# caoql98/LKGD

Hardware: AMD Instinct MI355X
Metric: denoised frames/sec (14f x 576x1024, 25-step Euler) (higher is better)
Workload: dtype f16; 1 GPU; SVD 14 frames x 576x1024, 25 Euler steps, CFG 1.0->3.0, single clip, vanilla pipeline_stable_video_diffusion_trans loop (configs[1]); unet=random-init SVD shapes (320,640,1280,1280), heads (5,10,20,20), 1.52 B params, parallelism=single GPU

## Files before the change

### lkgd_amd/csrc/gemm_wide.hip

```cpp
#include "gemm_common.h"

#ifdef WIDE_X_NOSTORE
#define WIDE_STORE_GUARD if (p.ldc < 0)
#elif defined(WIDE_X_ONELANE)
#define WIDE_STORE_GUARD if ((threadIdx.x & 63) == 0)
#else
#define WIDE_STORE_GUARD
#endif
#ifdef WIDE_X_SMALLOUT
#define WIDE_OUT_ROW(m) ((m) & 2047)
#else
#define WIDE_OUT_ROW(m) (m)
#endif
#ifdef WIDE_X_SMALLA
#define WIDE_A_ROW(m) ((m) & 4095)
#else
#define WIDE_A_ROW(m) (m)
#endif
#ifdef WIDE_X_NT
#define WIDE_ST(ptr, v) __builtin_nontemporal_store(v, ptr)
#else
#define WIDE_ST(ptr, v) (*(ptr) = (v))
#endif
#define WIDE_OUT_PITCH 336
#define WBM 256
#define WBN 320
#define WNT 512
#define WSTAGE_BYTES ((WBM + WBN) * BK * 2)
#define WBIAS_OFF (2 * WSTAGE_BYTES)
#define WRB_OFF (WBIAS_OFF + 2 * WBN * 4)
#define WRB_STRIP 768
#define WLDS (WRB_OFF + 4 * WRB_STRIP)

#define WIDE_WAIT_TOP "s_waitcnt lgkmcnt(0)\n\t"
#ifdef WIDE_X_NOSTAGE
#define WIDE_LD(X) ""
#else
#define WIDE_LD(X) X
#endif
#ifdef WIDE_X_NOREAD
#define WIDE_RD(X) ""
#else
#define WIDE_RD(X) X
#endif
#ifdef WIDE_X_NOMFMA
#define WIDE_MM(X) ""
#else
#define WIDE_MM(X) X
#endif
#if defined(WIDE_X_NOBAR) || defined(WIDE_X_STAMPS)
#define WIDE_BAR(X) ""
#else
#define WIDE_BAR(X) X
#endif
#include "gemm_wide_ktile.inc"

struct WideIn {
  unsigned oB[5];
  const half_t* wk;
};

template <bool FIRST, int NF, int MF>
__device__ __forceinline__ void wide_ktile_a(half8_t (&x1)[4], half8_t& w0, int xa0, int xa1, int wa0, int wa1,
                                             const half_t* const (&pA)[4], const WideIn& in, int m_a) {
  half8_t x0, x1_, x2, x3, w1;
#define WIDE_STMT(BODY)                                                                                                \
  asm volatile(BODY                                                                                                    \
               : "=&v"(x0), "=&v"(x1_), "=&v"(x2), "=&v"(x3), "=&v"(x1[0]), "=&v"(x1[1]), "=&v"(x1[2]), "=&v"(x1[3]),  \
                 "=&v"(w0), "=&v"(w1)                                                                                  \
               : "v"(xa0), "v"(xa1), "v"(wa0), "v"(wa1), "v"(pA[0]), "v"(pA[1]), "v"(pA[2]), "v"(pA[3]),               \
                 "v"(in.oB[0]), "v"(in.oB[1]), "v"(in.oB[2]), "v"(in.oB[3]), "v"(in.oB[4]), "s"(in.wk), "s"(m_a)       \
               : "memory", "scc", WIDE_AGPR_CLOBBERS)
  if (MF == 3) {
    if (NF == 8) {
      if (FIRST) {
        WIDE_STMT(WIDE8_M3_KTILE_ASM_FIRST_A);
      } else {
        WIDE_STMT(WIDE8_M3_KTILE_ASM_NEXT_A);
      }
    } else if (FIRST) {
      WIDE_STMT(WIDE_M3_KTILE_ASM_FIRST_A);
    } else {
      WIDE_STMT(WIDE_M3_KTILE_ASM_NEXT_A);
    }
  } else if (NF == 8) {
    if (FIRST) {
      WIDE_STMT(WIDE8_KTILE_ASM_FIRST_A);
    } else {
      WIDE_STMT(WIDE8_KTILE_ASM_NEXT_A);
    }
  } else if (FIRST) {
    WIDE_STMT(WIDE_KTILE_ASM_FIRST_A);
  } else {
    WIDE_STMT(WIDE_KTILE_ASM_NEXT_A);
  }
#undef WIDE_STMT
}

template <int NF, int MF>
__device__ __forceinline__ void wide_ktile_b(const half8_t (&x1)[4], half8_t w0, int wa1) {
  half8_t w1;
#define WIDE_STMT_B(BODY)                                                  \
  asm volatile(BODY                                                        \
               : "=&v"(w1), "+v"(w0)                                       \
               : "v"(x1[0]), "v"(x1[1]), "v"(x1[2]), "v"(x1[3]), "v"(wa1)  \
               : "memory", WIDE_AGPR_CLOBBERS)
  if (MF == 3) {
    if (NF == 8) WIDE_STMT_B(WIDE8_M3_KTILE_ASM_B);
    else WIDE_STMT_B(WIDE_M3_KTILE_ASM_B);
  } else if (NF == 8)
    asm volatile(WIDE8_KTILE_ASM_B
                 : "=&v"(w1), "+v"(w0)
                 : "v"(x1[0]), "v"(x1[1]), "v"(x1[2]), "v"(x1[3]), "v"(wa1)
                 : "memory", WIDE_AGPR_CLOBBERS);
  else
    asm volatile(WIDE_KTILE_ASM_B
                 : "=&v"(w1), "+v"(w0)
                 : "v"(x1[0]), "v"(x1[1]), "v"(x1[2]), "v"(x1[3]), "v"(wa1)
                 : "memory", WIDE_AGPR_CLOBBERS);
#undef WIDE_STMT_B
}

template <int BASE>
__device__ __forceinline__ float4_t wide_read_acc() {
  float a, b, c, d;
  asm volatile("v_accvgpr_read_b32 %0, a[%4]\n\tv_accvgpr_read_b32 %1, a[%4+1]\n\t"
               "v_accvgpr_read_b32 %2, a[%4+2]\n\tv_accvgpr_read_b32 %3, a[%4+3]"
               : "=v"(a), "=v"(b), "=v"(c), "=v"(d)
               : "i"(BASE));
  return (float4_t){a, b, c, d};
}

template <int V> struct WideIC { static constexpr int value = V; };
template <class F, int... Is> __device__ __forceinline__ void wide_static_for(F&& f, WideIC<Is>...) { (f(WideIC<Is>{}), ...); }
template <class F> __device__ __forceinline__ void wide_for10(F&& f) {
  wide_static_for(f, WideIC<0>{}, WideIC<1>{}, WideIC<2>{}, WideIC<3>{}, WideIC<4>{}, WideIC<5>{}, WideIC<6>{}, WideIC<7>{}, WideIC<8>{}, WideIC<9>{});
}
template <class F> __device__ __forceinline__ void wide_for8(F&& f) {
  wide_static_for(f, WideIC<0>{}, WideIC<1>{}, WideIC<2>{}, WideIC<3>{}, WideIC<4>{}, WideIC<5>{}, WideIC<6>{}, WideIC<7>{});
}
template <int NF, class F> __device__ __forceinline__ void wide_for_nf(F&& f) {
  if constexpr (NF == 8) wide_for8(f);
  else wide_for10(f);
}
template <class F> __device__ __forceinline__ void wide_for5(F&& f) {
  wide_static_for(f, WideIC<0>{}, WideIC<1>{}, WideIC<2>{}, WideIC<3>{}, WideIC<4>{});
}

template <int MODE, bool SPLIT, bool LDSOUT, int NF, int MF>
__device__ __forceinline__ void wide_body(const lkgd_gemm_desc& p, int tiles_m, int tiles_n, int ksplit_arg, float* ws) {
  static_assert(NF == 10 || (NF == 8 && !SPLIT), "wave tiles: 64 x 160 or 64 x 128 (the latter unsliced)");
  static_assert(MF == 4 || (MF == 3 && !SPLIT), "wave tiles: 64 or 48 rows (the latter unsliced)");
  constexpr int WM = 64 * MF;
  constexpr int WRW = 16 * MF;
  constexpr int WN = 32 * NF;
  constexpr int WCH = 16 * NF;
  const int ksplit = SPLIT ? ksplit_arg : 1;
  extern __shared__ __attribute__((aligned(16))) char smem[];
  const int t = threadIdx.x;
  const int lane = t & 63;
  const int w = __builtin_amdgcn_readfirstlane(t >> 6);
  const int wr = w >> 1, wc = w & 1;
  const int l15 = lane & 15, lq = lane >> 4;

  const int ntiles = tiles_m * tiles_n * ksplit;
  const int G = gridDim.x;
  const int xcd = blockIdx.x & 7, c = blockIdx.x >> 3;
  const int nc = (G - xcd + 7) >> 3;
  const int q8 = ntiles >> 3, r8 = ntiles & 7;
  const int xb = xcd * q8 + (xcd < r8 ? xcd : r8);
  const int xe = xb + q8 + (xcd < r8 ? 1 : 0);
  const int my_tiles = (xe - xb - c + nc - 1) / nc;
  const int tile_begin = xb + c;
  const int nk = p.K / BK / ksplit;
  const int total = (my_tiles > 0 ? my_tiles : 0) * nk;
  if (total <= 0) return;
  if (w >= 4) __builtin_amdgcn_s_setprio(1);
#ifdef WIDE_X_STAGGER
  for (int i = 0; i < (c & 3) * WIDE_X_STAGGER; ++i) __builtin_amdgcn_s_sleep(127);
#endif

  const int srow = t >> 3;
  const int schunk = (t & 7) ^ ((t >> 4) & 7);
  LeanGather<4> ag;
  float rcp0, rcp1;
  lean_rcps<MODE>(p, rcp0, rcp1);
  int st_tile = tile_begin - nc, st_kt = nk - 1, st_s = -1, st_par = 0, ep_par = 0;
  int st_k0 = 0;
  ag.seg_k0 = 0; ag.seg_end = 0; ag.zmask = 0; ag.ky = 0; ag.kx = 0; ag.cc = 0;
#pragma unroll
  for (int i = 0; i < 4; ++i) { ag.rd[i].base = -1; ag.rd[i].yx = 0; ag.aptr[i] = (const half_t*)p.zeros; }
  WideIn in;
#pragma unroll
  for (int i = 0; i < 5; ++i) in.oB[i] = 0;
  const bool rb_lds = p.rowbias && p.rb_d2 == 1 && p.rb_d1 >= WBM;
  const half_t* wbase = (const half_t*)p.w;
  asm volatile("" : "+s"(wbase));
  auto next_in = [&](WideIn& in) {
    if (st_s + 1 < total) {
      ++st_s;
      if (++st_kt == nk) {
        st_kt = 0;
        st_tile += nc;
        int tm, tn;
        supertile<4>(st_tile / ksplit, tiles_m, tiles_n, tm, tn);
        st_k0 = SPLIT ? (st_tile % ksplit) * nk : 0;
#pragma unroll
        for (int i = 0; i < MF; ++i) ag.rd[i] = lean_row<MODE>(p, WIDE_A_ROW(tm * WM) + srow + 64 * i, rcp0, rcp1);
#pragma unroll
        for (int i = 0; i < NF / 2; ++i) {
          int n = tn * WN + srow + 64 * i;
          n = n < p.N ? n : p.N - 1;
          in.oB[i] = ((unsigned)n * (unsigned)p.K + schunk * 8) * 2u;
        }
        ag.seg_end = 0;
        st_par ^= 1;
        if (p.bias && w < NF / 2) {
          int n = tn * WN + w * 64 + lane;
          n = n < p.N ? n : p.N - 1;
          __builtin_amdgcn_global_load_lds(GLB_PTR(p.bias + n), LDS_PTR(smem + WBIAS_OFF + st_par * (WBN * 4) + w * 256), 4, 0, 0);
        }
        if (rb_lds && w >= 5) {
          const unsigned mf = (unsigned)(tm * WM);
          unsigned ml = mf + WM - 1;
          ml = ml < (unsigned)p.M ? ml : (unsigned)p.M - 1;
          const unsigned i0 = ((mf / (unsigned)p.rb_d1) * (unsigned)p.rb_m1 + (unsigned)p.rb_c0) % (unsigned)p.rb_md;
          const unsigned i1 = ((ml / (unsigned)p.rb_d1) * (unsigned)p.rb_m1 + (unsigned)p.rb_c0) % (unsigned)p.rb_md;
          int dw = (w - 5) * 64 + lane;
          int col = tn * WN + 2 * (dw < WN / 2 ? dw : WN / 2 - 1);
          col = col < p.N - 2 ? col : p.N - 2;
          char* dst = smem + WRB_OFF + st_par * (2 * WRB_STRIP) + (w - 5) * 256;
          const half_t* rb = (const half_t*)p.rowbias;
          __builtin_amdgcn_global_load_lds(GLB_PTR(rb + (long long)i0 * p.ldrb + col), LDS_PTR(dst), 4, 0, 0);
          __builtin_amdgcn_global_load_lds(GLB_PTR(rb + (long long)i1 * p.ldrb + col), LDS_PTR(dst + WRB_STRIP), 4, 0, 0);
        }
      }
      if ((st_k0 + st_kt) * BK >= ag.seg_end) {
        lean_segment<MODE, 4>(p, ag, (st_k0 + st_kt) * BK, schunk);
        const int into = SPLIT ? (st_k0 + st_kt) * BK - ag.seg_k0 : 0;
        if (SPLIT && into) {
#pragma unroll
          for (int i = 0; i < 4; ++i) ag.aptr[i] += ((ag.zmask >> i) & 1u) ? 0 : into;
        }
      } else {
#pragma unroll
        for (int i = 0; i < 4; ++i) ag.aptr[i] += ((ag.zmask >> i) & 1u) ? 0 : BK;
      }
    }
    in.wk = wbase + (st_k0 + st_kt) * BK;
  };

  const int skey = (l15 >> 1) & 7;
  int xa0, xa1, wa0, wa1;
  {
    const int x_base = (wr * WRW + l15) * 128;
    const int w_base = WBM * BK * 2 + (wc * WCH + l15) * 128;
    const int ch0 = ((0 + lq) ^ skey) << 4, ch1 = ((4 + lq) ^ skey) << 4;
    xa0 = x_base + ch0; xa1 = x_base + ch1; wa0 = w_base + ch0; wa1 = w_base + ch1;
  }

  {
    next_in(in);
    char* sx = smem + w * 1024;
#pragma unroll
    for (int i = 0; i < MF; ++i) glds16(ag.aptr[i], sx + 8192 * i);
#pragma unroll
    for (int i = 0; i < NF / 2; ++i) glds16((const half_t*)((const char*)in.wk + in.oB[i]), sx + WBM * BK * 2 + 8192 * i);
  }
  next_in(in);

  int cur = 0, kt = 0, tile = tile_begin;
  bool skip_wait = false;
#ifdef WIDE_X_STAMPS
  long long st_sync = 0, st_body = 0, st_epi = 0, st_t0 = __builtin_amdgcn_s_memtime(), st_a, st_b;
#endif
#ifdef WIDE_X_LATEWAIT
  int late = 0;
#endif
#pragma unroll 1
  for (int s = 0; s < total; ++s) {
#ifdef WIDE_X_LATEWAIT
    if (late == 1) { asm volatile("s_waitcnt vmcnt(20)" ::: "memory"); skip_wait = true; }
    late = skip_wait && late == 0 ? 1 : 0;
#endif
#ifdef WIDE_X_STAMPS
    st_a = __builtin_amdgcn_s_memtime();
#endif
    if (!skip_wait) asm volatile("s_waitcnt vmcnt(0)" ::: "memory");
    skip_wait = false;
#ifdef WIDE_X_STAMPS
    __builtin_amdgcn_s_barrier();
    st_b = __builtin_amdgcn_s_memtime(); st_sync += st_b - st_a;
#endif
    const int m_a = (cur ^ 1) * WSTAGE_BYTES + w * 1024;
    half8_t x1[4], w0;
    if (kt == 0) wide_ktile_a<true, NF, MF>(x1, w0, xa0, xa1, wa0, wa1, ag.aptr, in, m_a);
    else wide_ktile_a<false, NF, MF>(x1, w0, xa0, xa1, wa0, wa1, ag.aptr, in, m_a);
    const int wa1_now = wa1;
    next_in(in);
    wide_ktile_b<NF, MF>(x1, w0, wa1_now);
    {
      const int d = cur ? -WSTAGE_BYTES : WSTAGE_BYTES;
      xa0 += d; xa1 += d; wa0 += d; wa1 += d;
    }
    cur ^= 1;
#ifdef WIDE_X_STAMPS
    st_a = __builtin_amdgcn_s_memtime(); st_body += st_a - st_b;
#endif

    if (++kt == nk) {
      asm volatile("s_waitcnt vmcnt(0)\n\ts_nop 15\n\ts_nop 15" ::: "memory");
      skip_wait = true;
      kt = 0;
      int lane_e = lane;
      asm volatile("" : "+v"(lane_e));
      const int l15 = lane_e & 15, lq = lane_e >> 4;
      int tm, tn;
      supertile<4>(tile / ksplit, tiles_m, tiles_n, tm, tn);
      const int slice = tile % ksplit;
      tile += nc;
      const int m0 = tm * WM + wr * WRW + l15;
      const int n0 = tn * WN + wc * WCH + 4 * lq;
      const half_t* rbp = (const half_t*)p.rowbias;
      const half_t* r1p = (const half_t*)p.res1;
      const half_t* r2p = (const half_t*)p.res2;
      half_t* outp = (half_t*)p.out;
      ep_par ^= 1;
      const float* bl = (const float*)(smem + WBIAS_OFF + ep_par * (WBN * 4)) + wc * WCH + 4 * lq;
      const half_t* rbl = (const half_t*)(smem + WRB_OFF + ep_par * (2 * WRB_STRIP)) + wc * WCH + 4 * lq;
      const unsigned rb_bound = rb_lds ? ((unsigned)(tm * WM) / (unsigned)p.rb_d1 + 1u) * (unsigned)p.rb_d1 : 0u;
      constexpr bool lds_out = LDSOUT && !SPLIT;
      char* scr = smem + (cur ^ 1) * WSTAGE_BYTES + w * (16 * WIDE_OUT_PITCH);
      if (lds_out) __builtin_amdgcn_s_barrier();
      const bool cs_on = lds_out && p.colstats != nullptr;
      float csum[2] = {0.f, 0.f}, csq[2] = {0.f, 0.f};
      auto epi = [&](auto jc) {
        constexpr int j = decltype(jc)::value;
        const long long m = m0 + j * 16;
        const bool live = m < p.M;
        if (!lds_out && !live) return;
        if (SPLIT) {
          float* dst = ws + ((long long)slice * p.M + m) * p.N;
          wide_for_nf<NF>([&](auto ic) {
            constexpr int i = decltype(ic)::value;
            const float4_t ev = wide_read_acc<(4 * i + j) * 4>();
            if (n0 + i * 16 < p.N) *(float4_t*)(dst + n0 + i * 16) = ev;
          });
          return;
        }
        const bool gg = NF == 10 && MODE == LKGD_A_PLAIN && !lds_out && p.geglu;
        if (!gg) {
          unsigned idx = 0;
          if (rbp && !rb_lds && live) idx = (((unsigned)m / (unsigned)p.rb_d1) * (unsigned)p.rb_m1 + ((unsigned)m % (unsigned)p.rb_d2) +
                                             (unsigned)p.rb_c0) % (unsigned)p.rb_md;
          const int rb_sel = (unsigned)m < rb_bound ? 0 : WRB_STRIP / 2;
          wide_for_nf<NF>([&](auto ic) {
            constexpr int i = decltype(ic)::value;
            const int n = n0 + i * 16;
            float4_t v = wide_read_acc<(4 * i + j) * 4>();
            if (n < p.N) {
              if (p.bias) v += *(const float4_t*)(bl + i * 16);
              if (rbp && live) {
                const half4_t rb = rb_lds ? *(const half4_t*)(rbl + rb_sel + i * 16)
                                          : *(const half4_t*)(rbp + (long long)idx * p.ldrb + n);
#pragma unroll
                for (int x = 0; x < 4; ++x) v[x] += (float)rb[x];
              }
              v *= p.s_acc;
              if (r1p && live) {
                half4_t r = *(const half4_t*)(r1p + m * p.ldr1 + n);
#pragma unroll
                for (int x = 0; x < 4; ++x) v[x] += p.r1 * (float)r[x];
              }
              if (r2p && live) {
                half4_t r = *(const half4_t*)(r2p + m * p.ldr2 + n);
#pragma unroll
                for (int x = 0; x < 4; ++x) v[x] += p.r2 * (float)r[x];
              }
              half4_t o;
#pragma unroll
              for (int x = 0; x < 4; ++x) o[x] = (half_t)v[x];
              if (lds_out) *(half4_t*)(scr + l15 * WIDE_OUT_PITCH + (i * 16 + 4 * lq) * 2) = o;
              else { WIDE_STORE_GUARD WIDE_ST((half4_t*)(outp + WIDE_OUT_ROW(m) * p.ldc + n), o); }
            }
          });
        } else {
          const int oc0 = tn * 160 + wc * 80 + 4 * lq;
          wide_for5([&](auto ic) {
            constexpr int i = decltype(ic)::value;
            float4_t hv = wide_read_acc<(4 * i + j) * 4>(), gv = wide_read_acc<(4 * (i + 5) + j) * 4>();
            if (p.bias) {
              hv += *(const float4_t*)(bl + i * 16);
              gv += *(const float4_t*)(bl + 80 + i * 16);
            }
#ifdef WIDE_X_NOGELU
            const float2_t lo = __builtin_shufflevector(hv, hv, 0, 1) * __builtin_shufflevector(gv, gv, 0, 1);
            const float2_t hi = __builtin_shufflevector(hv, hv, 2, 3) * __builtin_shufflevector(gv, gv, 2, 3);
#else
            const float2_t lo = __builtin_shufflevector(hv, hv, 0, 1) * gelu_erf2(__builtin_shufflevector(gv, gv, 0, 1));
            const float2_t hi = __builtin_shufflevector(hv, hv, 2, 3) * gelu_erf2(__builtin_shufflevector(gv, gv, 2, 3));
#endif
            const half4_t o = {(half_t)lo.x, (half_t)lo.y, (half_t)hi.x, (half_t)hi.y};
            if (lds_out) *(half4_t*)(scr + l15 * WIDE_OUT_PITCH + (i * 16 + 4 * lq) * 2) = o;
            else { WIDE_STORE_GUARD WIDE_ST((half4_t*)(outp + WIDE_OUT_ROW(m) * p.ldc + oc0 + i * 16), o); }
          });
        }
        if (lds_out) {
          const int per = gg ? 10 : 2 * NF;
          const long long mrow0 = (long long)tm * WM + wr * WRW + j * 16;
          if (cs_on && lane_e < 4 * NF) {
            const long long left = (long long)p.M - mrow0;
            const int nrows = left >= 16 ? 16 : (left > 0 ? (int)left : 0);
            #pragma unroll
            for (int r0 = 0; r0 < 16; r0 += 8) {
              half4_t u[8];
#pragma unroll
              for (int r = 0; r < 8; ++r) u[r] = *(const half4_t*)(scr + (r0 + r) * WIDE_OUT_PITCH + lane_e * 8);
#pragma unroll
              for (int r = 0; r < 8; ++r) {
                const half_t one = r0 + r < nrows ? (half_t)1.0f : (half_t)0.0f;
                const half2_t w2 = {one, one};
                const half2_t p0 = {u[r][0], u[r][1]}, p1 = {u[r][2], u[r][3]};
                csum[0] = __builtin_amdgcn_fdot2(p0, w2, csum[0], false);
                csum[1] = __builtin_amdgcn_fdot2(p1, w2, csum[1], false);
                csq[0] = __builtin_amdgcn_fdot2(p0, p0 * w2, csq[0], false);
                csq[1] = __builtin_amdgcn_fdot2(p1, p1 * w2, csq[1], false);
              }
            }
          }
          const int ncol0 = gg ? tn * 160 + wc * 80 : tn * WN + wc * WCH;
#pragma unroll
          for (int kk = 0; kk < 5; ++kk) {
            const int c = lane_e + 64 * kk;
            if (c < 16 * per) {
              const int row = NF == 8 ? c >> 4 : (gg ? (c * 205) >> 11 : (c * 205) >> 12);
              const int cc = c - row * per;
              const half8_t v = *(const half8_t*)(scr + row * WIDE_OUT_PITCH + cc * 16);
              const long long mr = mrow0 + row;
              if (mr < p.M) { WIDE_STORE_GUARD WIDE_ST((half8_t*)(outp + WIDE_OUT_ROW(mr) * p.ldc + ncol0 + cc * 8), v); }
            }
          }
        }
      };
#define WIDE_EPI(J)                                                                                                \
  {                                                                                                                \
    epi(WideIC<J>{});                                                                                              \
    __builtin_amdgcn_sched_barrier(0);     \
  }
      WIDE_EPI(0) WIDE_EPI(1) WIDE_EPI(2)
      if constexpr (MF == 4) WIDE_EPI(3)
#undef WIDE_EPI
      if (cs_on) {
        float* part = (float*)(smem + (cur ^ 1) * WSTAGE_BYTES + 8 * 16 * WIDE_OUT_PITCH);
        if (lane_e < 4 * NF)
          *(float4_t*)(part + (wr * (WN / 2) + wc * (WCH / 2) + 2 * lane_e) * 2) = (float4_t){csum[0], csq[0], csum[1], csq[1]};
        __builtin_amdgcn_s_barrier();
        if (t < WN / 2) {
          float a = 0.f, b = 0.f;
#pragma unroll
          for (int g = 0; g < 4; ++g) { a += part[(g * (WN / 2) + t) * 2]; b += part[(g * (WN / 2) + t) * 2 + 1]; }
          typedef float float2v __attribute__((ext_vector_type(2)));
          *(float2v*)(p.colstats + ((long long)tm * (p.N / 2) + tn * (WN / 2) + t) * 2) = (float2v){a, b};
        }
      }
#ifdef WIDE_X_STAMPS
      st_epi += __builtin_amdgcn_s_memtime() - st_a;
#endif
    }
  }
  asm volatile("s_waitcnt vmcnt(0)" ::: "memory");
#ifdef WIDE_X_STAMPS
  if (lane == 0) {
    long long* dbg = (long long*)p.out + ((long long)blockIdx.x * 8 + w) * 4;
    dbg[0] = st_sync; dbg[1] = st_body; dbg[2] = st_epi; dbg[3] = __builtin_amdgcn_s_memtime() - st_t0;
  }
#endif
}

template <int MODE, bool LDSOUT, int NF = 10, int MF = 4>
__global__ __launch_bounds__(WNT, 2) __attribute__((amdgpu_num_vgpr(96))) void lkgd_gemm_wide_kernel(const lkgd_gemm_desc p, int tiles_m, int tiles_n) {
  wide_body<MODE, false, LDSOUT, NF, MF>(p, tiles_m, tiles_n, 1, nullptr);
}
template <int MODE>
__global__ __launch_bounds__(WNT, 2) __attribute__((amdgpu_num_vgpr(96))) void lkgd_gemm_wide_split_kernel(const lkgd_gemm_desc p, int tiles_m, int tiles_n, int ksplit, float* ws) {
  wide_body<MODE, true, false, 10, 4>(p, tiles_m, tiles_n, ksplit, ws);
}

static thread_local int wide_lds_out_override = -1;
extern "C" void lkgd_debug_set_wide_lds_out(int on) { wide_lds_out_override = on; }

static thread_local int wide_tile_n_forced = 0;
extern "C" void lkgd_debug_set_wide_tile_n(int wn) { wide_tile_n_forced = (wn == 256 || wn == 320) ? wn : 0; }
extern "C" int lkgd_debug_wide_tile_n_forced() { return wide_tile_n_forced; }
static thread_local int wide_tile_m_forced = 0;
extern "C" void lkgd_debug_set_wide_tile_m(int wm) { wide_tile_m_forced = (wm == 192 || wm == 256) ? wm : 0; }
extern "C" int lkgd_debug_wide_tile_m_forced() { return wide_tile_m_forced; }
extern "C" int lkgd_gemm_wide_tile_n(int N) {
  if (wide_tile_n_forced && N % wide_tile_n_forced == 0) return wide_tile_n_forced;
  return (N % WBN != 0 && N % 256 == 0 && (long long)((N + WBN - 1) / WBN) * WBN * 10 > (long long)N * 11) ? 256 : WBN;
}

template <int MODE>
static void wide_go(const lkgd_gemm_desc* d, hipStream_t stream, int grid, int tiles_m, int tiles_n, bool lds_out, int wn, int wm) {
#define WIDE_GO(...) \
  hipLaunchKernelGGL((lkgd_gemm_wide_kernel<MODE, __VA_ARGS__>), dim3(grid), dim3(WNT), WLDS, stream, *d, tiles_m, tiles_n)
  if (wm == 192) {
    if (wn == 256) { if (lds_out) WIDE_GO(true, 8, 3); else WIDE_GO(false, 8, 3); }
    else { if (lds_out) WIDE_GO(true, 10, 3); else WIDE_GO(false, 10, 3); }
  } else {
    if (wn == 256) { if (lds_out) WIDE_GO(true, 8, 4); else WIDE_GO(false, 8, 4); }
    else { if (lds_out) WIDE_GO(true, 10, 4); else WIDE_GO(false, 10, 4); }
  }
#undef WIDE_GO
}
template <int MODE>
static bool wide_set_lds(const void* split_fn) {
  const void* fns[] = {(const void*)lkgd_gemm_wide_kernel<MODE, false, 10, 4>, (const void*)lkgd_gemm_wide_kernel<MODE, true, 10, 4>,
                       (const void*)lkgd_gemm_wide_kernel<MODE, false, 8, 4>,  (const void*)lkgd_gemm_wide_kernel<MODE, true, 8, 4>,
                       (const void*)lkgd_gemm_wide_kernel<MODE, false, 10, 3>, (const void*)lkgd_gemm_wide_kernel<MODE, true, 10, 3>,
                       (const void*)lkgd_gemm_wide_kernel<MODE, false, 8, 3>,  (const void*)lkgd_gemm_wide_kernel<MODE, true, 8, 3>, split_fn};
  for (const void* f : fns)
    if (hipFuncSetAttribute(f, hipFuncAttributeMaxDynamicSharedMemorySize, WLDS) != hipSuccess) return false;
  return true;
}

extern "C" int lkgd_gemm_wide_lds_out(const lkgd_gemm_desc* d, int ksplit, int wn) {
  const bool lds_ok = ksplit == 1 && !d->geglu && d->N % wn == 0 && d->ldc % 8 == 0 && aligned16(d->out);
  if (d->colstats && !lds_ok) return LKGD_E_SHAPE;
  return lds_ok && (d->colstats ? true : (wide_lds_out_override != 0 && d->mode == LKGD_A_PLAIN)) ? 1 : 0;
}

extern "C" int lkgd_gemm_wide_launch(const lkgd_gemm_desc* d, hipStream_t stream, int cus, int ksplit, int wn, int wm) {
  LKGD_DEVICE_ONCE_BEGIN
    if (!wide_set_lds<LKGD_A_PLAIN>((const void*)lkgd_gemm_wide_split_kernel<LKGD_A_PLAIN>) ||
        !wide_set_lds<LKGD_A_CONV3X3>((const void*)lkgd_gemm_wide_split_kernel<LKGD_A_CONV3X3>) ||
        !wide_set_lds<LKGD_A_TCONV3>((const void*)lkgd_gemm_wide_split_kernel<LKGD_A_TCONV3>))
      return LKGD_E_LAUNCH;
  LKGD_DEVICE_ONCE_END
  if ((wn != 256 && wn != WBN) || (wm != 192 && wm != WBM)) return LKGD_E_SHAPE;
  int tiles_m = (d->M + wm - 1) / wm, tiles_n = (d->N + wn - 1) / wn;
  if (ksplit < 1 || (d->K / BK) % ksplit || (ksplit > 1 && (!d->workspace || d->geglu))) return LKGD_E_SHAPE;
  if ((wn == 256 || wm == 192) && ksplit > 1) return LKGD_E_SHAPE;
  if (wn == 256 && d->geglu) return LKGD_E_SHAPE;
  long long ntiles = (long long)tiles_m * tiles_n * ksplit;
  if (ntiles > 0x7fffffffLL) return LKGD_E_SHAPE;
  int grid = ntiles < cus ? (int)ntiles : cus;
  if (d->M >= (1 << 24)) return LKGD_E_SHAPE;
  float* ws = (float*)d->workspace;
  const int lo = lkgd_gemm_wide_lds_out(d, ksplit, wn);
  if (lo < 0) return lo;
  const bool lds_out = lo != 0;
#define WIDE_LAUNCH(MODE_)                                                                                              \
  {                                                                                                                     \
    if (ksplit > 1)                                                                                                     \
      hipLaunchKernelGGL(lkgd_gemm_wide_split_kernel<MODE_>, dim3(grid), dim3(WNT), WLDS, stream, *d, tiles_m, tiles_n, ksplit, ws); \
    else                                                                                                                \
      wide_go<MODE_>(d, stream, grid, tiles_m, tiles_n, lds_out, wn, wm);                                               \
  }
  if (d->mode == LKGD_A_PLAIN) WIDE_LAUNCH(LKGD_A_PLAIN)
  else if (d->mode == LKGD_A_CONV3X3) WIDE_LAUNCH(LKGD_A_CONV3X3)
  else if (d->mode == LKGD_A_TCONV3) WIDE_LAUNCH(LKGD_A_TCONV3)
#undef WIDE_LAUNCH
  else
    return LKGD_E_MODE;
  return hipGetLastError() == hipSuccess ? LKGD_OK : LKGD_E_LAUNCH;
}
```

Measured before the change: 6.232 frames/s.

## Prefetch residual rows into freed accumulator registers during GEMM epilogue

The epilogue now issues the residual (res1) loads for the first row-fragment up front, and prefetches later row-fragments' residuals into AGPR accumulator slots that have already been consumed. Explicit s_waitcnt vmcnt counts, computed at compile time from the issue order, let each read wait only for its own load. This hides global-load latency of the residual add behind epilogue math instead of stalling on each load. The cost is fragile hand-counted vmcnt bookkeeping and inline asm that depends on AGPR slot reuse; partial tiles fall back to a full vmcnt(0) wait.

```diff
diff --git a/lkgd_amd/csrc/gemm_wide.hip b/lkgd_amd/csrc/gemm_wide.hip
--- a/lkgd_amd/csrc/gemm_wide.hip
+++ b/lkgd_amd/csrc/gemm_wide.hip
@@ -131,6 +131,57 @@
   return (float4_t){a, b, c, d};
 }
 
+__device__ __forceinline__ half4_t wide_res_load(const half_t* src) {
+  half4_t r;
+  asm volatile("global_load_dwordx2 %0, %1, off" : "=v"(r) : "v"(src) : "memory");
+  return r;
+}
+template <int REG>
+__device__ __forceinline__ void wide_res_prefetch(const half_t* src) {
+  static_assert(REG % 2 == 0 && REG >= 0 && REG + 1 < 160, "an even-aligned pair inside the accumulators");
+  asm volatile("global_load_dwordx2 a[%1:%2], %0, off" : : "v"(src), "i"(REG), "i"(REG + 1) : "memory");
+}
+template <int REG, int BEHIND>
+__device__ __forceinline__ half4_t wide_res_take(bool exact) {
+  typedef unsigned uint2v __attribute__((ext_vector_type(2)));
+  unsigned lo, hi;
+  if (exact)
+    asm volatile("s_waitcnt vmcnt(%2)\n\tv_accvgpr_read_b32 %0, a[%3]\n\tv_accvgpr_read_b32 %1, a[%4]"
+                 : "=v"(lo), "=v"(hi) : "i"(BEHIND), "i"(REG), "i"(REG + 1) : "memory");
+  else
+    asm volatile("s_waitcnt vmcnt(0)\n\tv_accvgpr_read_b32 %0, a[%2]\n\tv_accvgpr_read_b32 %1, a[%3]"
+                 : "=v"(lo), "=v"(hi) : "i"(REG), "i"(REG + 1) : "memory");
+  return __builtin_bit_cast(half4_t, ((uint2v){lo, hi}));
+}
+template <int NF>
+__device__ __forceinline__ void wide_res_landed(half4_t (&q)[NF], bool exact) {
+  static_assert(NF == 10 || NF == 8, "operand lists below");
+  if (exact) asm volatile("s_waitcnt vmcnt(2)" ::: "memory");
+  else asm volatile("s_waitcnt vmcnt(0)" ::: "memory");
+  if constexpr (NF == 10)
+    asm volatile("" : "+v"(q[0]), "+v"(q[1]), "+v"(q[2]), "+v"(q[3]), "+v"(q[4]), "+v"(q[5]), "+v"(q[6]), "+v"(q[7]), "+v"(q[8]), "+v"(q[9]) : : "memory");
+  else
+    asm volatile("" : "+v"(q[0]), "+v"(q[1]), "+v"(q[2]), "+v"(q[3]), "+v"(q[4]), "+v"(q[5]), "+v"(q[6]), "+v"(q[7]) : : "memory");
+}
+constexpr int wide_res_behind(int lds_stores, int NF, int MF, int ti, int tj) {
+  int pos = 0, want = 0;
+  for (int j = 0; j < MF; ++j) {
+    if (j == 0) pos += NF;
+    for (int i = 0; i < NF; ++i) {
+      if (j == 0) {
+        pos += 1; if (i == ti && tj == 1) want = pos;
+        pos += 1; if (i == ti && tj == 2) want = pos;
+      } else if (j == 1 && MF == 4) {
+        pos += 1; if (i == ti && tj == 3) want = pos;
+      }
+      if (i == ti && j == tj) return pos - want < 63 ? pos - want : 63;
+      if (!lds_stores) pos += 1;
+    }
+    pos += lds_stores;
+  }
+  return 0;
+}
+
 template <int V> struct WideIC { static constexpr int value = V; };
 template <class F, int... Is> __device__ __forceinline__ void wide_static_for(F&& f, WideIC<Is>...) { (f(WideIC<Is>{}), ...); }
 template <class F> __device__ __forceinline__ void wide_for10(F&& f) {
@@ -334,6 +385,13 @@
       if (lds_out) __builtin_amdgcn_s_barrier();
       const bool cs_on = lds_out && p.colstats != nullptr;
       float csum[2] = {0.f, 0.f}, csq[2] = {0.f, 0.f};
+      const bool res_on = !SPLIT && r1p;
+      constexpr int res_lds_stores = lds_out ? NF / 2 : 0;
+#ifdef WIDE_X_NOSTORE
+      const bool res_exact = false;
+#else
+      const bool res_exact = tm * WM + wr * WRW + WRW <= p.M && tn * WN + wc * WCH + WCH <= p.N;
+#endif
       auto epi = [&](auto jc) {
         constexpr int j = decltype(jc)::value;
         const long long m = m0 + j * 16;
@@ -354,10 +412,30 @@
           if (rbp && !rb_lds && live) idx = (((unsigned)m / (unsigned)p.rb_d1) * (unsigned)p.rb_m1 + ((unsigned)m % (unsigned)p.rb_d2) +
                                              (unsigned)p.rb_c0) % (unsigned)p.rb_md;
           const int rb_sel = (unsigned)m < rb_bound ? 0 : WRB_STRIP / 2;
+          half4_t q1[NF];
+          if constexpr (j == 0) {
+            if (r1p && live)
+              wide_for_nf<NF>([&](auto ic) {
+                constexpr int i = decltype(ic)::value;
+                if (n0 + i * 16 < p.N) q1[i] = wide_res_load(r1p + m * p.ldr1 + n0 + i * 16);
+              });
+          }
           wide_for_nf<NF>([&](auto ic) {
             constexpr int i = decltype(ic)::value;
             const int n = n0 + i * 16;
             float4_t v = wide_read_acc<(4 * i + j) * 4>();
+            if (res_on && n < p.N) {
+              constexpr int slot = (4 * i + j) * 4;
+              if constexpr (j == 0) {
+                if (m + 16 < p.M) wide_res_prefetch<slot>(r1p + (m + 16) * p.ldr1 + n);
+                if (m + 32 < p.M) wide_res_prefetch<slot + 2>(r1p + (m + 32) * p.ldr1 + n);
+              } else if constexpr (j == 1 && MF == 4) {
+                if (m + 32 < p.M) wide_res_prefetch<slot>(r1p + (m + 32) * p.ldr1 + n);
+              }
+            }
+            if constexpr (j == 0 && i == 0) {
+              if (res_on) wide_res_landed<NF>(q1, res_exact);
+            }
             if (n < p.N) {
               if (p.bias) v += *(const float4_t*)(bl + i * 16);
               if (rbp && live) {
@@ -367,8 +445,11 @@
                 for (int x = 0; x < 4; ++x) v[x] += (float)rb[x];
               }
               v *= p.s_acc;
+              constexpr int res_reg = j == 3 ? (4 * i + 1) * 4 : (4 * i) * 4 + (j == 2 ? 2 : 0);
               if (r1p && live) {
-                half4_t r = *(const half4_t*)(r1p + m * p.ldr1 + n);
+                half4_t r;
+                if constexpr (j == 0) r = q1[i];
+                else r = wide_res_take<res_reg, wide_res_behind(res_lds_stores, NF, MF, i, j)>(res_exact);
 #pragma unroll
                 for (int x = 0; x < 4; ++x) v[x] += p.r1 * (float)r[x];
               }
```

After: 6.247 frames/s (median of 6 runs). About the same (+0.2%).
